# M-Igashi/mp3rgain

Measured on AMD Instinct MI355X. Metric: stereo PCM samples/s through IIR+RMS+histogram, higher is better.
Workload: dtype f64

## Files before the change

mp3rgain_amd/csrc/rg_k2_tm.hip:

```cpp
#include <hip/hip_runtime.h>

#include <atomic>
#include <type_traits>

#include "rg_device.h"
#include "rg_device_inl.h"

#include "rg_tm.h"

namespace {

__device__ __forceinline__ double tm_step(double (&s)[10], double (&t)[2], const double x, const RgTmCoef &K) {
    const double y = fma(K.b[0], x, s[0]);
#pragma unroll
    for (int i = 0; i < 9; ++i) s[i] = fma(-K.a[i + 1], y, fma(K.b[i + 1], x, s[i + 1]));
    s[9] = fma(-K.a[10], y, fma(K.b[10], x, K.c0));
    const double z = fma(K.bb[0], y, t[0]);
    t[0] = fma(-K.ba[1], z, fma(K.bb[1], y, t[1]));
    t[1] = fma(-K.ba[2], z, fma(K.bb[2], y, K.c0));
    return z;
}

__device__ __forceinline__ double tm_step_servo(double (&s)[10], double (&t)[2], const double x, const RgTmCoef &K) {
    const double y = fma(K.b[0], x, s[0]);
#pragma unroll
    for (int i = 0; i < 9; ++i) s[i] = fma(-K.a[i + 1], y, fma(K.b[i + 1], x, s[i + 1]));
    s[9] = fma(-K.a[10], y, K.b[10] * x);
    const double z = y - t[0];
    const double p = t[0] + t[1];
    t[1] = fma(K.beta, z, t[1]);
    t[0] = fma(K.alpha, z, p);
    return z;
}

template <int NCH>
struct TmLane {
    double s[NCH][10];
    double t[NCH][2];
    double A[NCH];
    double B[NCH][RG_TM_DIM];
};

typedef __attribute__((address_space(4))) const double rg_cdouble;

template <int NCH, int NX>
__device__ __forceinline__ void tm_sample(TmLane<NCH> &st, const double (&x)[NCH], rg_cdouble *__restrict__ Trow,
                                          const RgTmCoef &K) {
#pragma unroll
    for (int c = 0; c < NCH; ++c) {
        const double z = tm_step(st.s[c], st.t[c], x[c], K);
        st.A[c] = fma(z, z, st.A[c]);
#pragma unroll
        for (int j = RG_TM_DIM - NX; j < RG_TM_DIM; ++j) st.B[c][j] = fma(z, Trow[j], st.B[c][j]);
    }
}

template <int FMT> struct Fmt;
template <> struct Fmt<RG_FMT_F32_PLANAR> {
    typedef float elem;
    typedef float peak_t;
    static __device__ __forceinline__ double cvt(float v, float &pk) { pk = fmaxf(pk, fabsf(v)); return (double)v; }
    static __device__ __forceinline__ double peak_norm(float pk) { return (double)pk; }
    static __device__ __forceinline__ float peak_denorm(double v) { return (float)v; }
    static __device__ __forceinline__ uint32_t word(float v) { return __float_as_uint(v); }
    static __device__ __forceinline__ double cvt_word(uint32_t w, float &pk) { return cvt(__uint_as_float(w), pk); }
    static __device__ __forceinline__ void peak4(const uint32_t (&f)[4], float &pk) {
        pk = fmaxf(fmaxf(pk, fabsf(__uint_as_float(f[0]))), fabsf(__uint_as_float(f[1])));
        pk = fmaxf(fmaxf(pk, fabsf(__uint_as_float(f[2]))), fabsf(__uint_as_float(f[3])));
    }
    static __device__ __forceinline__ double word_value(uint32_t w) { return (double)__uint_as_float(w); }
};
template <> struct Fmt<RG_FMT_S16_PLANAR> {
    typedef int16_t elem;
    typedef uint32_t peak_t;
    static __device__ __forceinline__ double cvt(int16_t v, uint32_t &pk) {
        const int32_t w = v;
        const uint32_t m = (uint32_t)(w < 0 ? -w : w);
        pk = m > pk ? m : pk;
        return (double)w;
    }
    static __device__ __forceinline__ double peak_norm(uint32_t pk) { return (double)pk / 32768.0; }
    static __device__ __forceinline__ uint32_t peak_denorm(double v) { return (uint32_t)(v * 32768.0); }
    static __device__ __forceinline__ uint32_t word(int16_t v) { return (uint32_t)(int32_t)v; }
    static __device__ __forceinline__ double cvt_word(uint32_t w, uint32_t &pk) { return cvt((int16_t)(int32_t)w, pk); }
    static __device__ __forceinline__ void peak4(const uint32_t (&f)[4], uint32_t &pk) {
#pragma unroll
        for (int u = 0; u < 4; ++u) (void)cvt_word(f[u], pk);
    }
    static __device__ __forceinline__ double word_value(uint32_t w) { return (double)(int32_t)w; }
};
template <> struct Fmt<RG_FMT_S32_PLANAR> {
    typedef int32_t elem;
    typedef uint32_t peak_t;
    static __device__ __forceinline__ double cvt(int32_t v, uint32_t &pk) {
        const uint32_t m = v < 0 ? (uint32_t)0 - (uint32_t)v : (uint32_t)v;
        pk = m > pk ? m : pk;
        return (double)v;
    }
    static __device__ __forceinline__ double peak_norm(uint32_t pk) { return (double)pk / 2147483648.0; }
    static __device__ __forceinline__ uint32_t peak_denorm(double v) { return (uint32_t)(v * 2147483648.0); }
    static __device__ __forceinline__ uint32_t word(int32_t v) { return (uint32_t)v; }
    static __device__ __forceinline__ double cvt_word(uint32_t w, uint32_t &pk) { return cvt((int32_t)w, pk); }
    static __device__ __forceinline__ void peak4(const uint32_t (&f)[4], uint32_t &pk) {
#pragma unroll
        for (int u = 0; u < 4; ++u) (void)cvt_word(f[u], pk);
    }
    static __device__ __forceinline__ double word_value(uint32_t w) { return (double)(int32_t)w; }
};

template <typename T>
__device__ __forceinline__ uint32_t find_track(const RgTmTrack *__restrict__ tracks, uint32_t n_tracks, uint32_t block,
                                               T RgTmTrack::*base) {
    uint32_t lo = 0, hi = n_tracks - 1;
    while (lo < hi) {
        const uint32_t mid = (lo + hi + 1) >> 1;
        if (tracks[mid].*base <= block) lo = mid; else hi = mid - 1;
    }
    return lo;
}

}

#define RG_TM_TILE 16

typedef uint32_t __attribute__((ext_vector_type(4))) rg_u32x4;
typedef uint32_t __attribute__((ext_vector_type(4), aligned(4))) rg_u32x4u;
typedef short __attribute__((ext_vector_type(4), aligned(2))) rg_s16x4u;

template <int FMT, int NX, bool MASK, bool PEAK = true, bool SERVO = false>
__device__ __forceinline__ void tm_frame(TmLane<1> &st, const uint32_t wbits, typename Fmt<FMT>::peak_t &pk,
                                         const double *__restrict__ tr , const RgTmCoef &K,
                                         const uint32_t n, const uint32_t len) {
    double (&s)[10] = st.s[0];
    double (&t)[2] = st.t[0];
    const double x = PEAK ? Fmt<FMT>::cvt_word(wbits, pk) : Fmt<FMT>::word_value(wbits);
#ifdef RG_TM_LOADER_ONLY
    st.A[0] += x;
    return;
#endif
    if constexpr (SERVO) {
        const double y = fma(K.b[0], x, s[0]);
        double u[10];
#pragma unroll
        for (int i = 0; i < 9; ++i) u[i] = fma(K.b[i + 1], x, s[i + 1]);
        u[9] = K.b[10] * x;
        const double p = t[0] + t[1];
        __builtin_amdgcn_sched_barrier(0);
        double z = y - t[0];
#pragma unroll
        for (int i = 0; i < 10; ++i) s[i] = fma(-K.a[i + 1], y, u[i]);
        __builtin_amdgcn_sched_barrier(0);
        if (MASK) z = n < len ? z : 0.0;
        t[1] = fma(K.beta, z, t[1]);
        t[0] = fma(K.alpha, z, p);
        st.A[0] = fma(z, z, st.A[0]);
#pragma unroll
        for (int j = 0; j < NX; ++j) st.B[0][RG_TM_DIM - NX + j] = fma(z, tr[j], st.B[0][RG_TM_DIM - NX + j]);
        __builtin_amdgcn_sched_barrier(0);
        return;
    }
    const double y = fma(K.b[0], x, s[0]);
    double u[10];
#pragma unroll
    for (int i = 0; i < 9; ++i) u[i] = fma(K.b[i + 1], x, s[i + 1]);
    u[9] = fma(K.b[10], x, K.c0);
    __builtin_amdgcn_sched_barrier(0);
    double z = fma(K.bb[0], y, t[0]);
    const double w1 = fma(K.bb[1], y, t[1]);
    const double w2 = fma(K.bb[2], y, K.c0);
    __builtin_amdgcn_sched_barrier(0);
#pragma unroll
    for (int i = 0; i < 10; ++i) s[i] = fma(-K.a[i + 1], y, u[i]);
    __builtin_amdgcn_sched_barrier(0);
    t[0] = fma(-K.ba[1], z, w1);
    t[1] = fma(-K.ba[2], z, w2);
    if (MASK) z = n < len ? z : 0.0;
    st.A[0] = fma(z, z, st.A[0]);
#pragma unroll
    for (int j = 0; j < NX; ++j) st.B[0][RG_TM_DIM - NX + j] = fma(z, tr[j], st.B[0][RG_TM_DIM - NX + j]);
    __builtin_amdgcn_sched_barrier(0);
}

template <int NX>
__device__ __forceinline__ void tm_load_row(double (&dst)[NX], const double *__restrict__ src) {
#pragma unroll
    for (int j = 0; j < NX; j += 2) {
        const double2 v = *reinterpret_cast<const double2 *>(src + j);
        dst[j] = v.x;
        dst[j + 1] = v.y;
    }
}

template <int FMT, bool TAIL, bool MOM, bool SERVO>
__device__ __forceinline__ void tm_fast_path(TmLane<1> &st, typename Fmt<FMT>::peak_t &pk, const RgTmCoef &K, const uint32_t L,
                                             const uint32_t H,
                                             const __attribute__((address_space(1))) typename Fmt<FMT>::elem *rowp,
                                             const uint32_t len,
                                             const double *__restrict__ T12, const double *__restrict__ T2,
                                             char *const wtile ) {
    typedef Fmt<FMT> F;
    typedef const __attribute__((address_space(1))) typename F::elem gelem;
    const int lane = threadIdx.x & 63;
#ifdef RG_TM_LINEWIDE
    constexpr bool kLineWide = !MOM && !TAIL && FMT == RG_FMT_F32_PLANAR;
#else
    constexpr bool kLineWide = false;
#endif
    const int lrow = lane >> 2, lslot = lane & 3;
    gelem *lfirst[4];
    uint32_t llen[4];
#pragma unroll
    for (int q = 0; q < 4; ++q) {
        const int row = 16 * q + lrow;
        const int piece = lslot ^ ((row >> 2) & 3);
        const unsigned long long base = __shfl((unsigned long long)(uintptr_t)rowp, row, 64);
        lfirst[q] = (gelem *)(uintptr_t)base + 4u * piece;
        llen[q] = L;
        if (TAIL) llen[q] = __shfl(len, row, 64);
    }
    const char *const rrow = wtile + lane * 64;
    const char *const rrow1 = wtile + RG_TM_WAVE_TILE_BYTES + (kLineWide ? lane ^ 1 : lane) * 64;
    const int rswz = (lane >> 2) & 3;
    const uint32_t ntiles = (L + RG_TM_TILE - 1) / RG_TM_TILE;

    constexpr int NSTAGE = MOM ? 1 : 2;
    rg_u32x4 stage[NSTAGE][4];
    auto load4 = [&](gelem *src) -> rg_u32x4 {
        if constexpr (FMT == RG_FMT_S16_PLANAR) {
            const rg_s16x4u v = *(const __attribute__((address_space(1))) rg_s16x4u *)src;
            return rg_u32x4{(uint32_t)(int32_t)v.x, (uint32_t)(int32_t)v.y, (uint32_t)(int32_t)v.z, (uint32_t)(int32_t)v.w};
        } else {
            return *(const __attribute__((address_space(1))) rg_u32x4u *)src;
        }
    };
    auto load_tile = [&](uint32_t tile, auto buf, auto whole) {
        constexpr int SB = decltype(buf)::value;
        constexpr bool WHOLE = decltype(whole)::value;
        const uint32_t n0 = tile * RG_TM_TILE;
#pragma unroll
        for (int q = 0; q < 4; ++q) {
            const int row = 16 * q + lrow;
            const int piece = lslot ^ ((row >> 2) & 3);
            const uint32_t pn = n0 + 4u * piece;
            if (!TAIL) {
                if (WHOLE || n0 + RG_TM_TILE <= L || pn < L) stage[SB][q] = load4(lfirst[q] + n0);
            } else {
                gelem *src = lfirst[q] + n0;
                if (pn + 4u <= llen[q]) {
                    stage[SB][q] = load4(src);
                } else {
                    stage[SB][q].x = pn + 0u < llen[q] ? F::word(src[0]) : 0u;
                    stage[SB][q].y = pn + 1u < llen[q] ? F::word(src[1]) : 0u;
                    stage[SB][q].z = pn + 2u < llen[q] ? F::word(src[2]) : 0u;
                    stage[SB][q].w = pn + 3u < llen[q] ? F::word(src[3]) : 0u;
                }
            }
        }
    };
    auto store_tile = [&](auto buf) {
        constexpr int SB = decltype(buf)::value;
        __builtin_amdgcn_wave_barrier();
#pragma unroll
        for (int q = 0; q < 4; ++q)
            *reinterpret_cast<uint4 *>(wtile + SB * RG_TM_WAVE_TILE_BYTES + q * 1024 + (lane ^ (kLineWide && SB ? 4 : 0)) * 16) =
                make_uint4(stage[SB][q].x, stage[SB][q].y, stage[SB][q].z, stage[SB][q].w);
        __builtin_amdgcn_fence(__ATOMIC_RELEASE, "wavefront");
        __builtin_amdgcn_wave_barrier();
    };
    auto read_piece = [&](int p, int slot) -> uint4 { return *reinterpret_cast<const uint4 *>((slot ? rrow1 : rrow) + 16 * (p ^ rswz)); };

    auto compute_tile = [&](const uint32_t tile, auto mode, auto buf) {
        constexpr int MODE = decltype(mode)::value;
        constexpr int SLOT = decltype(buf)::value;
        const uint32_t n0 = tile * RG_TM_TILE;
        const int np = (MODE != 0 && MODE != 4) ? 4 : (L - n0 >= RG_TM_TILE ? 4 : (int)((L - n0) >> 2));
        auto piece = [&](const int p, const uint4 v) {
            const uint32_t f[4] = {v.x, v.y, v.z, v.w};
            const uint32_t n = n0 + 4u * p;
            F::peak4(f, pk);
            if (MODE == 3 || MODE == 4) {
#pragma unroll
                for (int u = 0; u < 4; ++u) tm_frame<FMT, 0, TAIL, false, SERVO>(st, f[u], pk, nullptr, K, n + u, len);
            } else if (MODE == 1 || (MODE == 0 && n < H)) {
#pragma unroll
                for (int u = 0; u < 4; ++u) {
                    double row[12];
                    tm_load_row<12>(row, T12 + (size_t)(n + u) * 12);
                    tm_frame<FMT, 12, TAIL, false, SERVO>(st, f[u], pk, row, K, n + u, len);
                }
            } else {
                double rows[8];
                tm_load_row<4>(reinterpret_cast<double (&)[4]>(rows[0]), T2 + (size_t)(n - H) * 2);
                tm_load_row<4>(reinterpret_cast<double (&)[4]>(rows[4]), T2 + (size_t)(n - H) * 2 + 4);
#pragma unroll
                for (int u = 0; u < 4; ++u) {
                    const double tr[2] = {rows[2 * u], rows[2 * u + 1]};
                    tm_frame<FMT, 2, TAIL, false, SERVO>(st, f[u], pk, tr, K, n + u, len);
                }
            }
        };
        if constexpr (MODE != 0 && MODE != 4) {
            uint4 v[4];
            v[0] = read_piece(0, SLOT);
#pragma unroll
            for (int p = 0; p < 4; ++p) {
                if (p + 1 < 4) v[p + 1] = read_piece(p + 1, SLOT);
                piece(p, v[p]);
            }
        } else {
            uint4 v = make_uint4(0u, 0u, 0u, 0u);
            if (np) v = read_piece(0, SLOT);
#pragma unroll 1
            for (int p = 0; p < np; ++p) {
                const uint4 vn = p + 1 < np ? read_piece(p + 1, SLOT) : v;
                piece(p, v);
                v = vn;
            }
        }
        if ((MODE == 0 || MODE == 4) && tile + 1 == ntiles) {
            for (uint32_t n = L & ~3u; n < L; ++n) {
                const uint32_t o = n - n0;
                const uint32_t f = *reinterpret_cast<const uint32_t *>((SLOT ? rrow1 : rrow) + 16 * ((int)(o >> 2) ^ rswz) + 4 * (o & 3));
                if (MODE == 4) {
                    tm_frame<FMT, 0, TAIL, true, SERVO>(st, f, pk, nullptr, K, n, len);
                } else if (n < H) {
                    double row[12];
                    tm_load_row<12>(row, T12 + (size_t)n * 12);
                    tm_frame<FMT, 12, TAIL, true, SERVO>(st, f, pk, row, K, n, len);
                } else {
                    const double tr[2] = {T2[(size_t)(n - H) * 2], T2[(size_t)(n - H) * 2 + 1]};
                    tm_frame<FMT, 2, TAIL, true, SERVO>(st, f, pk, tr, K, n, len);
                }
            }
        }
    };
    typedef std::integral_constant<int, 0> Mixed;
    typedef std::integral_constant<int, 1> All12;
    typedef std::integral_constant<int, 2> All2;
    typedef std::integral_constant<int, 3> None;
    typedef std::integral_constant<int, 4> NoneRagged;

    typedef std::integral_constant<int, 0> S0;
    typedef std::integral_constant<int, NSTAGE - 1> S1;
    typedef std::false_type Guarded;
    typedef std::true_type Whole;
    auto run_tile = [&](const uint32_t tile, auto mode, auto buf) {
        store_tile(buf);
        if (tile + NSTAGE < ntiles) load_tile(tile + NSTAGE, buf, Guarded{});
        compute_tile(tile, mode, buf);
    };
    const uint32_t full_tiles = L / RG_TM_TILE;
    uint32_t tile = 0;
    if constexpr (MOM) load_tile(0, S0{}, Guarded{});
    if constexpr (!MOM) {
        if constexpr (kLineWide) {
            const int wrow = lane >> 3, wslot = (lane >> 2) & 1, wpos = lane & 3;
            unsigned long long lo64 = (unsigned long long)(uintptr_t)rowp;
#pragma unroll
            for (int d = 32; d >= 1; d >>= 1) {
                const unsigned long long o = __shfl_xor(lo64, d, 64);
                lo64 = o < lo64 ? o : lo64;
            }
            const unsigned long long wbase = __builtin_amdgcn_readfirstlane((uint32_t)lo64) | ((unsigned long long)__builtin_amdgcn_readfirstlane((uint32_t)(lo64 >> 32)) << 32);
            const unsigned long long delta = (unsigned long long)(uintptr_t)rowp - wbase;
            const bool near = __all(delta < (1ull << 31)) && full_tiles >= 4;
            if (near) {
                uint32_t woff[8];
#pragma unroll
                for (int q = 0; q < 8; ++q) {
                    const int row = 8 * q + wrow;
                    woff[q] = __shfl((uint32_t)delta, row, 64) + 64u * wslot + 16u * (wpos ^ ((row >> 2) & 3));
                }
                const __attribute__((address_space(1))) char *const gb = (const __attribute__((address_space(1))) char *)(uintptr_t)wbase;
                auto pair_load = [&](const uint32_t t0) {
#pragma unroll
                    for (int q = 0; q < 8; ++q)
                        stage[q >> 2][q & 3] = *(const __attribute__((address_space(1))) rg_u32x4u *)(gb + (size_t)t0 * (RG_TM_TILE * 4) + woff[q]);
                };
                auto pair_store = [&]() {
                    __builtin_amdgcn_wave_barrier();
#pragma unroll
                    for (int q = 0; q < 8; ++q)
                        *reinterpret_cast<uint4 *>(wtile + wslot * RG_TM_WAVE_TILE_BYTES + ((8 * q + wrow) ^ wslot) * 64 + wpos * 16) =
                            make_uint4(stage[q >> 2][q & 3].x, stage[q >> 2][q & 3].y, stage[q >> 2][q & 3].z, stage[q >> 2][q & 3].w);
                    __builtin_amdgcn_fence(__ATOMIC_RELEASE, "wavefront");
                    __builtin_amdgcn_wave_barrier();
                };
                pair_load(0);
                for (; tile + 3 < full_tiles; tile += 2) {
                    pair_store();
                    if (tile + 5 < full_tiles) {
                        pair_load(tile + 2);
                    } else {
                        load_tile(tile + 2, S0{}, Guarded{});
                        if (tile + 3 < ntiles) load_tile(tile + 3, S1{}, Guarded{});
                    }
                    compute_tile(tile, None{}, S0{});
                    compute_tile(tile + 1, None{}, S1{});
                }
            } else {
                load_tile(0, S0{}, Guarded{});
                if (ntiles > 1) load_tile(1, S1{}, Guarded{});
                for (; tile + 3 < full_tiles; tile += 2) {
                    store_tile(S0{});
                    store_tile(S1{});
                    load_tile(tile + 2, S0{}, Whole{});
                    load_tile(tile + 3, S1{}, Whole{});
                    compute_tile(tile, None{}, S0{});
                    compute_tile(tile + 1, None{}, S1{});
                }
            }
        } else {
        load_tile(0, S0{}, Guarded{});
        if (ntiles > 1) load_tile(1, S1{}, Guarded{});
        for (; tile + 3 < full_tiles; tile += 2) {
            store_tile(S0{});
            store_tile(S1{});
            load_tile(tile + 2, S0{}, Whole{});
            load_tile(tile + 3, S1{}, Whole{});
            compute_tile(tile, None{}, S0{});
            compute_tile(tile + 1, None{}, S1{});
        }
        }
        while (tile < ntiles) {
            if (tile < full_tiles) run_tile(tile, None{}, S0{}); else run_tile(tile, NoneRagged{}, S0{});
            if (++tile >= ntiles) break;
            if (tile < full_tiles) run_tile(tile, None{}, S1{}); else run_tile(tile, NoneRagged{}, S1{});
            ++tile;
        }
        return;
    }
    const uint32_t t12 = (H / RG_TM_TILE) < full_tiles ? H / RG_TM_TILE : full_tiles;
    for (; tile < t12; ++tile) run_tile(tile, All12{}, S0{});
    if (tile < ntiles && (tile * RG_TM_TILE < H || tile >= full_tiles)) { run_tile(tile, Mixed{}, S0{}); ++tile; }
    for (; tile < full_tiles; ++tile) run_tile(tile, All2{}, S0{});
    for (; tile < ntiles; ++tile) run_tile(tile, Mixed{}, S0{});
}

template <int FMT, bool MULTI, bool SERVO>
__global__ void __launch_bounds__(MULTI ? RG_TM_BLOCK_WIDE_MULTI : RG_TM_BLOCK_WIDE)
rg_tm_main_kernel(const RgTmCoef K, const RgTmGeom G, const RgTmTrack *__restrict__ tracks, uint32_t n_tracks,
                  double *__restrict__ rec, uint32_t total_recs, double *__restrict__ win_energy ,
                  uint32_t total_windows, uint32_t *__restrict__ nonfinite, uint32_t lds_tables,
                  uint32_t *__restrict__ zero_words, uint64_t zero_count ,
                  unsigned long long *__restrict__ dbg ) {
    typedef Fmt<FMT> F;
    const unsigned long long dbg_t0 = dbg ? wall_clock64() : 0ull;
    const unsigned long long dbg_c0 = dbg ? __builtin_readcyclecounter() : 0ull;
    typedef typename F::elem elem;
    typedef __attribute__((address_space(1))) const elem gelem;
    extern __shared__ __attribute__((aligned(16))) char smem[];

    if (zero_words) {
        const uint64_t stride = (uint64_t)gridDim.x * blockDim.x;
        for (uint64_t w = (uint64_t)blockIdx.x * blockDim.x + threadIdx.x; w < zero_count; w += stride) zero_words[w] = 0u;
    }
    const uint32_t gl = blockIdx.x * blockDim.x + threadIdx.x;
    const uint32_t t = find_track(tracks, n_tracks, gl, &RgTmTrack::lane_base);
    struct { const void *ch0, *ch1; uint64_t frames; uint32_t nseg; } tr;
    {
        const RgTmTrack &q = tracks[t];
        tr.ch0 = q.ch0; tr.ch1 = q.ch1; tr.frames = q.frames; tr.nseg = q.nseg;
    }
    const uint32_t rel = gl - tracks[t].lane_base;
    const int chan = (tr.ch1 != nullptr && rel >= tr.nseg) ? 1 : 0;
    const uint32_t seg = rel - (chan ? tr.nseg : 0u);
    const uint32_t L = G.L;
    const uint32_t H = G.H10;
    const uint32_t m = MULTI ? G.m : 1u;
    const uint64_t seg_stride = (uint64_t)L * m;
    const bool active = seg < tr.nseg;
    const uint64_t start = (uint64_t)seg * seg_stride;
    uint32_t len = 0;
    if (active) {
        const uint64_t rem = tr.frames - start;
        len = rem < L ? (uint32_t)rem : L;
    }
    gelem *const chp = (gelem *)(chan == 0 ? tr.ch0 : tr.ch1);
    rg_cdouble *__restrict__ T = (rg_cdouble *)G.T;

    TmLane<1> st;
#pragma unroll
    for (int i = 0; i < 10; ++i) st.s[0][i] = 0.0;
    st.t[0][0] = st.t[0][1] = 0.0;
    st.A[0] = 0.0;
#pragma unroll
    for (int j = 0; j < RG_TM_DIM; ++j) st.B[0][j] = 0.0;
    typename F::peak_t pk = 0;
    auto rec_ptr = [&]() -> double * { return rec + (size_t)chan * RG_TM_REC * total_recs + ((size_t)tracks[t].rec_base + (active ? seg : 0)); };
    auto note_nonfinite = [&](const double energy, const uint32_t unit, const bool counts) {
        const bool bad = counts && !(fabs(energy) <= 1.7976931348623157e308);
        if (__any(bad) && bad) atomicMax(&nonfinite[tracks[t].track_index], 0xFFFFFFFFu - unit);
    };

    auto first_energy = [&]() -> double {
        if constexpr (SERVO) return fabs(st.A[0]) <= 1.7976931348623157e308 ? st.A[0] + fma(K.aff_lin, st.t[0][1], K.aff_n * (double)len) : st.A[0];
        return st.A[0];
    };
    bool done = false;
    {
        if (lds_tables) {
            done = true;
            const uint32_t tbl_doubles = H * 12 + (L - H) * 2;
            {
                const double2 *__restrict__ src = reinterpret_cast<const double2 *>(G.Tlds);
                double2 *dst = reinterpret_cast<double2 *>(smem);
                const uint32_t n16 = tbl_doubles / 2;
                const uint32_t BS = blockDim.x;
                uint32_t i = threadIdx.x;
                for (; i + 3 * BS < n16; i += 4 * BS) {
                    const double2 a = src[i], b = src[i + BS], c = src[i + 2 * BS], d = src[i + 3 * BS];
                    dst[i] = a;
                    dst[i + BS] = b;
                    dst[i + 2 * BS] = c;
                    dst[i + 3 * BS] = d;
                }
                for (; i < n16; i += BS) dst[i] = src[i];
                __syncthreads();
            }
            const double *const T12 = reinterpret_cast<const double *>(smem);
            const double *const T2 = T12 + (size_t)H * 12;
            char *const wtile = smem + (size_t)tbl_doubles * sizeof(double) + (threadIdx.x >> 6) * (RG_TM_WAVE_TILE_BYTES * (MULTI ? 2 : 1));
            const bool plain = len == L && start + ((L + 3u) & ~3u) <= tr.frames;
            if (__all(plain))
                tm_fast_path<FMT, false, true, SERVO>(st, pk, K, L, H, chp + start, len, T12, T2, wtile);
            else if (__any(len != 0))
                tm_fast_path<FMT, true, true, SERVO>(st, pk, K, L, H, chp + start, len, T12, T2, wtile);
            if constexpr (MULTI) {
                note_nonfinite(st.A[0], seg * m, active);
                if (active) {
                    double *__restrict__ const r = rec_ptr();
                    r[0] = first_energy();
#pragma unroll
                    for (int j = 0; j < RG_TM_DIM; ++j) r[(size_t)(1 + j) * total_recs] = st.B[0][j];
                }
#pragma unroll 1
                for (uint32_t w = 1; w < m; ++w) {
                    const uint64_t wstart = start + (uint64_t)w * L;
                    uint32_t lenw = 0;
                    if (active && wstart < tr.frames) {
                        const uint64_t rem = tr.frames - wstart;
                        lenw = rem < L ? (uint32_t)rem : L;
                    }
                    if (!__any(lenw != 0)) break;
                    st.A[0] = 0.0;
                    const double v2_start = st.t[0][1];
                    const bool idle = lenw == 0 && tr.frames >= (uint64_t)((L + 3u) & ~3u);
                    const bool plainw = idle || (lenw == L && wstart + ((L + 3u) & ~3u) <= tr.frames);
                    gelem *const rowp = idle ? chp : chp + wstart;
                    if (__all(plainw))
                        tm_fast_path<FMT, false, false, SERVO>(st, pk, K, L, H, rowp, lenw, T12, T2, wtile);
                    else
                        tm_fast_path<FMT, true, false, SERVO>(st, pk, K, L, H, rowp, lenw, T12, T2, wtile);
                    note_nonfinite(st.A[0], seg * m + w, lenw != 0);
                    double energy = st.A[0];
                    if constexpr (SERVO) energy = fabs(energy) <= 1.7976931348623157e308 ? energy + fma(K.aff_lin, st.t[0][1] - v2_start, K.aff_n * (double)lenw) : energy;
                    if (lenw != 0) win_energy[(size_t)chan * total_windows + tracks[t].win_base + (size_t)seg * m + w] = energy;
                }
            }
        }
    }
    if (!done) {
        gelem *const p0 = chp + start;
        for (uint32_t n = 0; n < L; ++n) {
            const bool valid = n < len;
            double x = 0.0;
            if (valid) x = F::cvt(p0[n], pk);
            rg_cdouble *__restrict__ Trow = T + (size_t)n * RG_TM_DIM;
            double z;
            if constexpr (SERVO) {
                const double v2 = st.t[0][1];
                z = tm_step_servo(st.s[0], st.t[0], x, K);
                if (!valid) st.t[0][1] = v2;
            } else {
                z = tm_step(st.s[0], st.t[0], x, K);
            }
            z = valid ? z : 0.0;
            st.A[0] = fma(z, z, st.A[0]);
#pragma unroll
            for (int j = 0; j < RG_TM_DIM; ++j) st.B[0][j] = fma(z, Trow[j], st.B[0][j]);
        }
    }

    if (dbg && (threadIdx.x & 63) == 0) {
        const size_t w = ((size_t)blockIdx.x * (blockDim.x / 64) + (threadIdx.x >> 6)) * 6;
        dbg[w + 4] = dbg_c0;
        dbg[w + 5] = __builtin_readcyclecounter();
        dbg[w + 0] = dbg_t0;
        dbg[w + 1] = wall_clock64();
        dbg[w + 2] = ((unsigned long long)__builtin_amdgcn_s_getreg((20 << 0) | (0 << 6) | (31 << 11)) << 32) |
                     __builtin_amdgcn_s_getreg((4 << 0) | (0 << 6) | (31 << 11));
        dbg[w + 3] = done ? 1ull : 0ull;
    }

    if constexpr (!MULTI) {
        note_nonfinite(st.A[0], seg, active);
        if (active) {
            double *__restrict__ const r = rec_ptr();
            r[0] = first_energy();
#pragma unroll
            for (int j = 0; j < RG_TM_DIM; ++j) r[(size_t)(1 + j) * total_recs] = st.B[0][j];
        }
    }
    if (active) {
        double *__restrict__ const r = rec_ptr();
#pragma unroll
        for (int j = 0; j < 10; ++j) r[(size_t)(13 + j) * total_recs] = st.s[0][j];
        r[(size_t)23 * total_recs] = st.t[0][0];
        r[(size_t)24 * total_recs] = st.t[0][1];
        r[(size_t)25 * total_recs] = F::peak_norm(pk);
    }
}


template <typename V>
__device__ __forceinline__ void tm_performed(V old) {
    asm volatile("" ::"v"(old));
}

template <typename GP>
__device__ __forceinline__ double tm_quad_half(GP Gm, const double (&sg)[RG_TM_DIM]) {
    double quad = 0.0;
    int p = 0;
#pragma unroll
    for (int j = 0; j < RG_TM_DIM; ++j) {
        double row = 0.5 * Gm[p] * sg[j];
        ++p;
#pragma unroll
        for (int q = j + 1; q < RG_TM_DIM; ++q, ++p) row = fma(Gm[p], sg[q], row);
        quad = fma(row, sg[j], quad);
    }
    return quad;
}

template <int NCH>
__global__ void __launch_bounds__(RG_TM_BLOCK)
rg_tm_fix_kernel(const RgTmGeom G, const RgTmFixTables FT, const RgTmTrack *__restrict__ tracks, uint32_t n_tracks,
                 const double *__restrict__ rec, uint32_t total_recs,
                 const double *__restrict__ win_energy , uint32_t total_windows,
                 uint32_t *__restrict__ nonfinite,
                 uint32_t *__restrict__ imprecise, uint32_t *__restrict__ hist,
                 unsigned long long *__restrict__ peak_bits, uint32_t *__restrict__ done_count,
                 rg_track_result *__restrict__ results,
                 unsigned long long *__restrict__ dbg ) {
#define TM_FIX_STAMP(k)                                                            \
    do {                                                                           \
        if (dbg && threadIdx.x == 0) dbg[(size_t)blockIdx.x * 8 + (k)] = wall_clock64(); \
    } while (0)
    __builtin_amdgcn_s_setprio(3);
    TM_FIX_STAMP(0);
    __shared__ double edge[RG_TM_BLOCK / 64][RG_TM_EDGE][NCH * RG_TM_DIM];
    __shared__ uint64_t pct_scan[RG_PCT_THREADS];
    __shared__ double pieces[RG_TM_BLOCK];
    __shared__ double pieces_m[RG_TM_BLOCK];
    __shared__ double pieces_e[RG_TM_BLOCK];
    __shared__ int is_last;
    __shared__ double part_sg[NCH][RG_TM_DIM];
    __shared__ uint32_t part_len;
    __shared__ int part_lane;
    const int lane = threadIdx.x & 63, wave = threadIdx.x >> 6;
    if (threadIdx.x == 0) part_len = 0;
    auto publish_edge = [&](const double x, const int slot) {
        if (lane >= 64 - RG_TM_EDGE) edge[wave][lane - (64 - RG_TM_EDGE)][slot] = x;
    };
    auto from_below = [&](const double x, const int d, const int slot) -> double {
        double v = __shfl_up(x, d, 64);
        if (lane < d) v = wave > 0 ? edge[wave - 1][RG_TM_EDGE - d + lane][slot] : 0.0;
        return v;
    };

    const uint32_t t = find_track(tracks, n_tracks, blockIdx.x, &RgTmTrack::fix_block_base);
    const RgTmTrack tr = tracks[t];
    const uint32_t b = blockIdx.x - tr.fix_block_base;
    const int i = threadIdx.x;
    const int warm = (int)G.warm;
    const uint32_t NB = G.fix_windows * G.k;
    const long long seg = (long long)b * NB - warm + i;
    const bool in_block = i < warm + (int)NB;
    const bool seg_valid = in_block && seg >= 0 && seg < (long long)tr.nseg;
    const bool owner = seg_valid && i >= warm;
    const size_t idx = (size_t)tr.rec_base + (size_t)(seg_valid ? seg : 0);
    __shared__ double ftab[RG_TM_GRAM + RG_TM_MAX_ROUNDS * 104 + 36 + 100 + 12];
    {
        const double *__restrict__ src = FT.Gp + (size_t)(G.L - 1) * RG_TM_GRAM;
        const int n = RG_TM_GRAM + (int)G.rounds * 104 + 36 + (G.servo ? 112 : (G.whiten ? 100 : 0));
        for (int q = i; q < n; q += RG_TM_BLOCK) ftab[q] = src[q];
    }
    const double *const Gfull = ftab;
    const double *const PhiY = ftab + RG_TM_GRAM;
    const double *const PhiB = PhiY + G.rounds * 100;
    const double *const X = PhiB + G.rounds * 4;
    const double *const S0 = X + 24;
    const double *const Wf = S0 + 12;
    const double *const STf = Wf + 100;

    double w[NCH][RG_TM_DIM], pk = 0.0;
#pragma unroll
    for (int c = 0; c < NCH; ++c) {
        const double *__restrict__ r = rec + (size_t)c * RG_TM_REC * total_recs + idx;
#pragma unroll
        for (int j = 0; j < RG_TM_DIM; ++j) w[c][j] = seg_valid ? r[(size_t)(13 + j) * total_recs] : 0.0;
    }
    __syncthreads();
    TM_FIX_STAMP(1);
    const bool vstart = in_block && seg == -1;
#pragma unroll
    for (int c = 0; c < NCH; ++c) {
        double tq[2];
#pragma unroll
        for (int q = 0; q < 2; ++q) {
            double acc = G.whiten ? fma(X[q * 12 + 10], w[c][10], X[q * 12 + 11] * w[c][11]) : w[c][10 + q];
#pragma unroll
            for (int j = 0; j < 10; ++j) acc = fma(X[q * 12 + j], w[c][j], acc);
            tq[q] = acc;
        }
        w[c][10] = tq[0];
        w[c][11] = tq[1];
        if (G.whiten) {
#pragma unroll
            for (int i = 0; i < 10; ++i) {
                double acc = 0.0;
#pragma unroll
                for (int j = 0; j < 10; ++j)
                    if (j >= i) acc = fma(Wf[i * 10 + j], w[c][j], acc);
                w[c][i] = acc;
            }
        }
        if (vstart) {
#pragma unroll
            for (int j = 0; j < RG_TM_DIM; ++j) w[c][j] = S0[j];
        }
    }
    for (uint32_t rd = 0; rd < G.rounds; ++rd) {
        const int d = 1 << rd;
        const bool fast = rd < G.rounds_fast;
        double wn[NCH][RG_TM_DIM];
#pragma unroll
        for (int c = 0; c < NCH; ++c)
#pragma unroll
            for (int j = 0; j < RG_TM_DIM; ++j)
                if (j >= 10 || fast) publish_edge(w[c][j], c * RG_TM_DIM + j);
        __syncthreads();
#pragma unroll
        for (int c = 0; c < NCH; ++c)
#pragma unroll
            for (int j = 0; j < RG_TM_DIM; ++j) wn[c][j] = (j >= 10 || fast) ? from_below(w[c][j], d, c * RG_TM_DIM + j) : 0.0;
        __syncthreads();
        if (fast) {
            const double *PY = PhiY + (size_t)rd * 100;
#pragma unroll
            for (int a = 0; a < 10; ++a) {
                double py[10];
#pragma unroll
                for (int q = 0; q < 10; ++q) py[q] = PY[a * 10 + q];
#pragma unroll
                for (int c = 0; c < NCH; ++c) {
                    double acc = w[c][a];
#pragma unroll
                    for (int q = 0; q < 10; ++q) acc = fma(py[q], wn[c][q], acc);
                    w[c][a] = acc;
                }
                if (a & 1) __builtin_amdgcn_sched_barrier(0);
            }
        }
        const double *PB = PhiB + (size_t)rd * 4;
#pragma unroll
        for (int c = 0; c < NCH; ++c) {
            w[c][10] = fma(PB[0], wn[c][10], fma(PB[1], wn[c][11], w[c][10]));
            w[c][11] = fma(PB[2], wn[c][10], fma(PB[3], wn[c][11], w[c][11]));
        }
    }
#pragma unroll
    for (int c = 0; c < NCH; ++c)
#pragma unroll
        for (int j = 0; j < RG_TM_DIM; ++j) publish_edge(w[c][j], c * RG_TM_DIM + j);
    __syncthreads();
    double sgm[NCH][RG_TM_DIM];
#pragma unroll
    for (int c = 0; c < NCH; ++c)
#pragma unroll
        for (int j = 0; j < RG_TM_DIM; ++j) sgm[c][j] = from_below(w[c][j], 1, c * RG_TM_DIM + j);

    TM_FIX_STAMP(2);
    double S = 0.0, Mseg = 0.0, Eseg = 0.0;
    if (owner) {
        const uint64_t start = (uint64_t)seg * G.L * G.m;
        const uint64_t rem = tr.frames - start;
        const uint32_t len = rem < G.L ? (uint32_t)rem : G.L;
        const bool full = len == G.L;
        double lin[NCH], quad[NCH];
#pragma unroll
        for (int c = 0; c < NCH; ++c) {
            const double *__restrict__ r = rec + (size_t)c * RG_TM_REC * total_recs + idx;
            double acc = 0.0;
#pragma unroll
            for (int j = 0; j < RG_TM_DIM; ++j) acc = fma(r[(size_t)(1 + j) * total_recs], sgm[c][j], acc);
            lin[c] = acc;
            quad[c] = 0.0;
            pk = fmax(pk, r[(size_t)25 * total_recs]);
            S += r[0];
            Mseg += r[0];
            double st = 0.0;
#pragma unroll
            for (int j = 0; j < 10; ++j) st = fma(fabs(sgm[c][j]), G.tau10[j], st);
            Eseg = fma(2.0 * st, sqrt(fabs(r[0])) * 1.0001, Eseg);
        }
        if (full) {
#pragma unroll
            for (int j = 0; j < RG_TM_DIM; ++j) {
                const int p = j * RG_TM_DIM - (j * (j - 1)) / 2 - j;
                double g[RG_TM_DIM];
#pragma unroll
                for (int q = 0; q < RG_TM_DIM; ++q)
                    if (q >= j) g[q] = Gfull[p + q];
#pragma unroll
                for (int c = 0; c < NCH; ++c) {
                    double row = 0.5 * g[j] * sgm[c][j];
#pragma unroll
                    for (int q = 0; q < RG_TM_DIM; ++q)
                        if (q > j) row = fma(g[q], sgm[c][q], row);
                    quad[c] = fma(row, sgm[c][j], quad[c]);
                }
                __builtin_amdgcn_sched_barrier(0);
            }
        } else {
#pragma unroll
            for (int c = 0; c < NCH; ++c)
#pragma unroll
                for (int j = 0; j < RG_TM_DIM; ++j) part_sg[c][j] = sgm[c][j];
            part_len = len;
            part_lane = i;
        }
#pragma unroll
        for (int c = 0; c < NCH; ++c) {
            S += 2.0 * (lin[c] + quad[c]);
            Mseg += 2.0 * quad[c];
        }
        if (G.servo && full) {
            double aff = 0.0;
#pragma unroll
            for (int c = 0; c < NCH; ++c) {
                double sx = 0.0;
#pragma unroll
                for (int j = 0; j < RG_TM_DIM; ++j) sx = fma(STf[j], sgm[c][j], sx);
                aff = fma(G.aff_sig, sx, aff);
            }
            S += aff;
        }
    }
    const uint32_t nf = nonfinite[tr.track_index];
    if (nf != 0 && owner) {
        const uint64_t unit = (uint64_t)seg * G.m, bad = 0xFFFFFFFFu - nf;
        if (unit > bad) S = __longlong_as_double(0x7FF8000000000000ll);
        else if (unit == bad) {
            double cls = 0.0;
#pragma unroll
            for (int c = 0; c < NCH; ++c) {
                const double a = rec[(size_t)c * RG_TM_REC * total_recs + idx];
                if (!(fabs(a) <= 1.7976931348623157e308)) cls += a;
            }
// ... 214 lines not shown
```

Before: 452.5 billion.

## Stream follow-on windows continuously through one double-buffered tile pipeline

Replaces the per-window loop, which re-entered the tile pipeline for each window with its own prologue, drain and ragged tail, with a single streaming path that processes all subsequent windows of a segment as one continuous sample stream. Window boundaries and track ends are handled inside event tiles, and lanes whose tracks end are re-pinned to an idle pointer, so the steady loop keeps double-buffered whole-tile loads going across window edges. The fast path is simplified to the first-window momentum mode and the optional line-wide variant is removed. The cost is more complex boundary logic, with wave-wide votes and per-sample handling at window edges.

```diff
diff --git a/mp3rgain_amd/csrc/rg_k2_tm.hip b/mp3rgain_amd/csrc/rg_k2_tm.hip
--- a/mp3rgain_amd/csrc/rg_k2_tm.hip
+++ b/mp3rgain_amd/csrc/rg_k2_tm.hip
@@ -191,7 +191,7 @@
     }
 }
 
-template <int FMT, bool TAIL, bool MOM, bool SERVO>
+template <int FMT, bool TAIL, bool SERVO>
 __device__ __forceinline__ void tm_fast_path(TmLane<1> &st, typename Fmt<FMT>::peak_t &pk, const RgTmCoef &K, const uint32_t L,
                                              const uint32_t H,
                                              const __attribute__((address_space(1))) typename Fmt<FMT>::elem *rowp,
@@ -201,11 +201,6 @@
     typedef Fmt<FMT> F;
     typedef const __attribute__((address_space(1))) typename F::elem gelem;
     const int lane = threadIdx.x & 63;
-#ifdef RG_TM_LINEWIDE
-    constexpr bool kLineWide = !MOM && !TAIL && FMT == RG_FMT_F32_PLANAR;
-#else
-    constexpr bool kLineWide = false;
-#endif
     const int lrow = lane >> 2, lslot = lane & 3;
     gelem *lfirst[4];
     uint32_t llen[4];
@@ -219,11 +214,10 @@
         if (TAIL) llen[q] = __shfl(len, row, 64);
     }
     const char *const rrow = wtile + lane * 64;
-    const char *const rrow1 = wtile + RG_TM_WAVE_TILE_BYTES + (kLineWide ? lane ^ 1 : lane) * 64;
     const int rswz = (lane >> 2) & 3;
     const uint32_t ntiles = (L + RG_TM_TILE - 1) / RG_TM_TILE;
 
-    constexpr int NSTAGE = MOM ? 1 : 2;
+    constexpr int NSTAGE = 1;
     rg_u32x4 stage[NSTAGE][4];
     auto load4 = [&](gelem *src) -> rg_u32x4 {
         if constexpr (FMT == RG_FMT_S16_PLANAR) {
@@ -262,26 +256,23 @@
         __builtin_amdgcn_wave_barrier();
 #pragma unroll
         for (int q = 0; q < 4; ++q)
-            *reinterpret_cast<uint4 *>(wtile + SB * RG_TM_WAVE_TILE_BYTES + q * 1024 + (lane ^ (kLineWide && SB ? 4 : 0)) * 16) =
+            *reinterpret_cast<uint4 *>(wtile + SB * RG_TM_WAVE_TILE_BYTES + q * 1024 + lane * 16) =
                 make_uint4(stage[SB][q].x, stage[SB][q].y, stage[SB][q].z, stage[SB][q].w);
         __builtin_amdgcn_fence(__ATOMIC_RELEASE, "wavefront");
         __builtin_amdgcn_wave_barrier();
     };
-    auto read_piece = [&](int p, int slot) -> uint4 { return *reinterpret_cast<const uint4 *>((slot ? rrow1 : rrow) + 16 * (p ^ rswz)); };
+    auto read_piece = [&](int p, int) -> uint4 { return *reinterpret_cast<const uint4 *>(rrow + 16 * (p ^ rswz)); };
 
     auto compute_tile = [&](const uint32_t tile, auto mode, auto buf) {
         constexpr int MODE = decltype(mode)::value;
         constexpr int SLOT = decltype(buf)::value;
         const uint32_t n0 = tile * RG_TM_TILE;
-        const int np = (MODE != 0 && MODE != 4) ? 4 : (L - n0 >= RG_TM_TILE ? 4 : (int)((L - n0) >> 2));
+        const int np = MODE != 0 ? 4 : (L - n0 >= RG_TM_TILE ? 4 : (int)((L - n0) >> 2));
         auto piece = [&](const int p, const uint4 v) {
             const uint32_t f[4] = {v.x, v.y, v.z, v.w};
             const uint32_t n = n0 + 4u * p;
             F::peak4(f, pk);
-            if (MODE == 3 || MODE == 4) {
-#pragma unroll
-                for (int u = 0; u < 4; ++u) tm_frame<FMT, 0, TAIL, false, SERVO>(st, f[u], pk, nullptr, K, n + u, len);
-            } else if (MODE == 1 || (MODE == 0 && n < H)) {
+            if (MODE == 1 || (MODE == 0 && n < H)) {
 #pragma unroll
                 for (int u = 0; u < 4; ++u) {
                     double row[12];
@@ -299,7 +290,7 @@
                 }
             }
         };
-        if constexpr (MODE != 0 && MODE != 4) {
+        if constexpr (MODE != 0) {
             uint4 v[4];
             v[0] = read_piece(0, SLOT);
 #pragma unroll
@@ -317,13 +308,11 @@
                 v = vn;
             }
         }
-        if ((MODE == 0 || MODE == 4) && tile + 1 == ntiles) {
+        if (MODE == 0 && tile + 1 == ntiles) {
             for (uint32_t n = L & ~3u; n < L; ++n) {
                 const uint32_t o = n - n0;
-                const uint32_t f = *reinterpret_cast<const uint32_t *>((SLOT ? rrow1 : rrow) + 16 * ((int)(o >> 2) ^ rswz) + 4 * (o & 3));
-                if (MODE == 4) {
-                    tm_frame<FMT, 0, TAIL, true, SERVO>(st, f, pk, nullptr, K, n, len);
-                } else if (n < H) {
+                const uint32_t f = *reinterpret_cast<const uint32_t *>(rrow + 16 * ((int)(o >> 2) ^ rswz) + 4 * (o & 3));
+                if (n < H) {
                     double row[12];
                     tm_load_row<12>(row, T12 + (size_t)n * 12);
                     tm_frame<FMT, 12, TAIL, true, SERVO>(st, f, pk, row, K, n, len);
@@ -337,13 +326,9 @@
     typedef std::integral_constant<int, 0> Mixed;
     typedef std::integral_constant<int, 1> All12;
     typedef std::integral_constant<int, 2> All2;
-    typedef std::integral_constant<int, 3> None;
-    typedef std::integral_constant<int, 4> NoneRagged;
 
     typedef std::integral_constant<int, 0> S0;
-    typedef std::integral_constant<int, NSTAGE - 1> S1;
     typedef std::false_type Guarded;
-    typedef std::true_type Whole;
     auto run_tile = [&](const uint32_t tile, auto mode, auto buf) {
         store_tile(buf);
         if (tile + NSTAGE < ntiles) load_tile(tile + NSTAGE, buf, Guarded{});
@@ -351,90 +336,219 @@
     };
     const uint32_t full_tiles = L / RG_TM_TILE;
     uint32_t tile = 0;
-    if constexpr (MOM) load_tile(0, S0{}, Guarded{});
-    if constexpr (!MOM) {
-        if constexpr (kLineWide) {
-            const int wrow = lane >> 3, wslot = (lane >> 2) & 1, wpos = lane & 3;
-            unsigned long long lo64 = (unsigned long long)(uintptr_t)rowp;
-#pragma unroll
-            for (int d = 32; d >= 1; d >>= 1) {
-                const unsigned long long o = __shfl_xor(lo64, d, 64);
-                lo64 = o < lo64 ? o : lo64;
-            }
-            const unsigned long long wbase = __builtin_amdgcn_readfirstlane((uint32_t)lo64) | ((unsigned long long)__builtin_amdgcn_readfirstlane((uint32_t)(lo64 >> 32)) << 32);
-            const unsigned long long delta = (unsigned long long)(uintptr_t)rowp - wbase;
-            const bool near = __all(delta < (1ull << 31)) && full_tiles >= 4;
-            if (near) {
-                uint32_t woff[8];
-#pragma unroll
-                for (int q = 0; q < 8; ++q) {
-                    const int row = 8 * q + wrow;
-                    woff[q] = __shfl((uint32_t)delta, row, 64) + 64u * wslot + 16u * (wpos ^ ((row >> 2) & 3));
-                }
-                const __attribute__((address_space(1))) char *const gb = (const __attribute__((address_space(1))) char *)(uintptr_t)wbase;
-                auto pair_load = [&](const uint32_t t0) {
-#pragma unroll
-                    for (int q = 0; q < 8; ++q)
-                        stage[q >> 2][q & 3] = *(const __attribute__((address_space(1))) rg_u32x4u *)(gb + (size_t)t0 * (RG_TM_TILE * 4) + woff[q]);
-                };
-                auto pair_store = [&]() {
-                    __builtin_amdgcn_wave_barrier();
-#pragma unroll
-                    for (int q = 0; q < 8; ++q)
-                        *reinterpret_cast<uint4 *>(wtile + wslot * RG_TM_WAVE_TILE_BYTES + ((8 * q + wrow) ^ wslot) * 64 + wpos * 16) =
-                            make_uint4(stage[q >> 2][q & 3].x, stage[q >> 2][q & 3].y, stage[q >> 2][q & 3].z, stage[q >> 2][q & 3].w);
-                    __builtin_amdgcn_fence(__ATOMIC_RELEASE, "wavefront");
-                    __builtin_amdgcn_wave_barrier();
-                };
-                pair_load(0);
-                for (; tile + 3 < full_tiles; tile += 2) {
-                    pair_store();
-                    if (tile + 5 < full_tiles) {
-                        pair_load(tile + 2);
-                    } else {
-                        load_tile(tile + 2, S0{}, Guarded{});
-                        if (tile + 3 < ntiles) load_tile(tile + 3, S1{}, Guarded{});
-                    }
-                    compute_tile(tile, None{}, S0{});
-                    compute_tile(tile + 1, None{}, S1{});
-                }
-            } else {
-                load_tile(0, S0{}, Guarded{});
-                if (ntiles > 1) load_tile(1, S1{}, Guarded{});
-                for (; tile + 3 < full_tiles; tile += 2) {
-                    store_tile(S0{});
-                    store_tile(S1{});
-                    load_tile(tile + 2, S0{}, Whole{});
-                    load_tile(tile + 3, S1{}, Whole{});
-                    compute_tile(tile, None{}, S0{});
-                    compute_tile(tile + 1, None{}, S1{});
-                }
-            }
-        } else {
-        load_tile(0, S0{}, Guarded{});
-        if (ntiles > 1) load_tile(1, S1{}, Guarded{});
-        for (; tile + 3 < full_tiles; tile += 2) {
-            store_tile(S0{});
-            store_tile(S1{});
-            load_tile(tile + 2, S0{}, Whole{});
-            load_tile(tile + 3, S1{}, Whole{});
-            compute_tile(tile, None{}, S0{});
-            compute_tile(tile + 1, None{}, S1{});
-        }
-        }
-        while (tile < ntiles) {
-            if (tile < full_tiles) run_tile(tile, None{}, S0{}); else run_tile(tile, NoneRagged{}, S0{});
-            if (++tile >= ntiles) break;
-            if (tile < full_tiles) run_tile(tile, None{}, S1{}); else run_tile(tile, NoneRagged{}, S1{});
-            ++tile;
-        }
-        return;
-    }
+    load_tile(0, S0{}, Guarded{});
     const uint32_t t12 = (H / RG_TM_TILE) < full_tiles ? H / RG_TM_TILE : full_tiles;
     for (; tile < t12; ++tile) run_tile(tile, All12{}, S0{});
     if (tile < ntiles && (tile * RG_TM_TILE < H || tile >= full_tiles)) { run_tile(tile, Mixed{}, S0{}); ++tile; }
     for (; tile < full_tiles; ++tile) run_tile(tile, All2{}, S0{});
     for (; tile < ntiles; ++tile) run_tile(tile, Mixed{}, S0{});
+}
+
+template <int FMT, bool SERVO, typename GetPin, typename WindowDone>
+__device__ __forceinline__ void tm_stream_path(TmLane<1> &st, typename Fmt<FMT>::peak_t &pk, const RgTmCoef &K, const uint32_t L,
+                                               const uint32_t m,
+                                               const __attribute__((address_space(1))) typename Fmt<FMT>::elem *const sp ,
+                                               const uint32_t slen ,
+                                               GetPin &&get_pin ,
+                                               char *const wtile ,
+                                               WindowDone &&window_done ) {
+    typedef Fmt<FMT> F;
+    typedef const __attribute__((address_space(1))) typename F::elem gelem;
+    typedef const __attribute__((address_space(1))) char gbyte;
+    constexpr uint32_t EB = sizeof(typename F::elem);
+    constexpr uint32_t IDLE = 0xFFFFFFFFu;
+    const int lane = threadIdx.x & 63;
+    const uint32_t S = L * (m - 1);
+    auto is_live = [](const uint32_t v) { return v != 0u && v != IDLE; };
+    uint32_t vend = slen;
+    if (slen == 0) vend = get_pin() != nullptr ? IDLE : 0u;
+    bool any_dead = __any(vend == 0u);
+    const int lrow = lane >> 2, lslot = lane & 3;
+    gbyte *lptr[4];
+    uint32_t lstep[4];
+    uint32_t lt = 0;
+    {
+        gelem *const first = slen ? sp : get_pin();
+#pragma unroll
+        for (int q = 0; q < 4; ++q) {
+            const int row = 16 * q + lrow;
+            const int piece = lslot ^ ((row >> 2) & 3);
+            const unsigned long long base = __shfl((unsigned long long)(uintptr_t)first, row, 64);
+            lptr[q] = (gbyte *)(uintptr_t)base + 4u * EB * piece;
+            lstep[q] = __shfl(slen, row, 64) ? 2u * RG_TM_TILE * EB : 0u;
+        }
+    }
+    const char *const rrow = wtile + lane * 64;
+    const int rswz = (lane >> 2) & 3;
+
+    rg_u32x4 stage[2][4];
+    auto load4 = [&](gelem *src) -> rg_u32x4 {
+        if constexpr (FMT == RG_FMT_S16_PLANAR) {
+            const rg_s16x4u v = *(const __attribute__((address_space(1))) rg_s16x4u *)src;
+            return rg_u32x4{(uint32_t)(int32_t)v.x, (uint32_t)(int32_t)v.y, (uint32_t)(int32_t)v.z, (uint32_t)(int32_t)v.w};
+        } else {
+            return *(const __attribute__((address_space(1))) rg_u32x4u *)src;
+        }
+    };
+    auto load_tile = [&](auto dt, auto buf, auto whole) {
+        constexpr int DT = decltype(dt)::value;
+        constexpr int SB = decltype(buf)::value;
+        constexpr bool WHOLE = decltype(whole)::value;
+        const uint32_t n0 = (lt + DT) * RG_TM_TILE;
+        if (!WHOLE && n0 >= S) return;
+#pragma unroll
+        for (int q = 0; q < 4; ++q) {
+            gelem *const src = (gelem *)(lptr[q] + DT * RG_TM_TILE * EB);
+            if (WHOLE) {
+                stage[SB][q] = load4(src);
+            } else {
+                const int row = 16 * q + lrow;
+                const int piece = lslot ^ ((row >> 2) & 3);
+                const uint32_t pn = n0 + 4u * piece;
+                const uint32_t llen = __shfl(vend, row, 64);
+                if (pn + 4u <= llen) {
+                    stage[SB][q] = load4(src);
+                } else {
+                    stage[SB][q].x = pn + 0u < llen ? F::word(src[0]) : 0u;
+                    stage[SB][q].y = pn + 1u < llen ? F::word(src[1]) : 0u;
+                    stage[SB][q].z = pn + 2u < llen ? F::word(src[2]) : 0u;
+                    stage[SB][q].w = pn + 3u < llen ? F::word(src[3]) : 0u;
+                }
+            }
+        }
+    };
+    auto advance = [&]() {
+#pragma unroll
+        for (int q = 0; q < 4; ++q) lptr[q] += lstep[q];
+        lt += 2;
+    };
+    auto store_tile = [&](auto buf) {
+        constexpr int SB = decltype(buf)::value;
+        __builtin_amdgcn_wave_barrier();
+#pragma unroll
+        for (int q = 0; q < 4; ++q)
+            *reinterpret_cast<uint4 *>(wtile + SB * RG_TM_WAVE_TILE_BYTES + q * 1024 + lane * 16) =
+                make_uint4(stage[SB][q].x, stage[SB][q].y, stage[SB][q].z, stage[SB][q].w);
+        __builtin_amdgcn_fence(__ATOMIC_RELEASE, "wavefront");
+        __builtin_amdgcn_wave_barrier();
+    };
+    auto compute_tile = [&](auto buf) {
+        constexpr int SLOT = decltype(buf)::value;
+        const char *const r = rrow + SLOT * RG_TM_WAVE_TILE_BYTES;
+        uint4 v[4];
+        v[0] = *reinterpret_cast<const uint4 *>(r + 16 * (0 ^ rswz));
+#pragma unroll
+        for (int p = 0; p < 4; ++p) {
+            if (p + 1 < 4) v[p + 1] = *reinterpret_cast<const uint4 *>(r + 16 * ((p + 1) ^ rswz));
+            const uint32_t f[4] = {v[p].x, v[p].y, v[p].z, v[p].w};
+            F::peak4(f, pk);
+#pragma unroll
+            for (int u = 0; u < 4; ++u) tm_frame<FMT, 0, false, false, SERVO>(st, f[u], pk, nullptr, K, 0u, 0u);
+        }
+    };
+
+    uint32_t w = 1;
+    uint32_t wbase = 0;
+    uint32_t bnext = L;
+    st.A[0] = 0.0;
+    double v2_start = st.t[0][1];
+
+    auto event_tile = [&](const uint32_t tile, const int slot) -> bool {
+        const uint32_t n0 = tile * RG_TM_TILE;
+        const char *const r = rrow + slot * RG_TM_WAVE_TILE_BYTES;
+        uint32_t o = 0;
+#pragma unroll 1
+        while (o < RG_TM_TILE) {
+            const uint32_t n = n0 + o;
+            if (n >= S) return true;
+            if ((o & 3u) == 0u && bnext >= n + 4u && __all(vend >= n + 4u)) {
+                const uint4 v = *reinterpret_cast<const uint4 *>(r + 16 * ((int)(o >> 2) ^ rswz));
+                const uint32_t f[4] = {v.x, v.y, v.z, v.w};
+                F::peak4(f, pk);
+#pragma unroll
+                for (int u = 0; u < 4; ++u) tm_frame<FMT, 0, false, false, SERVO>(st, f[u], pk, nullptr, K, 0u, 0u);
+                o += 4u;
+            } else {
+                const uint32_t f = *reinterpret_cast<const uint32_t *>(r + 16 * ((int)(o >> 2) ^ rswz) + 4 * (o & 3u));
+                tm_frame<FMT, 0, true, true, SERVO>(st, f, pk, nullptr, K, n, vend);
+                o += 1u;
+            }
+            if (n0 + o == bnext) {
+                const uint32_t rem = vend - wbase;
+                window_done(w, rem < L ? rem : L, is_live(vend) && vend > wbase, v2_start);
+                st.A[0] = 0.0;
+                v2_start = st.t[0][1];
+                wbase = bnext;
+                bnext += L;
+                if (++w == m) return true;
+            }
+        }
+        const bool ends = is_live(vend) && vend <= n0 + RG_TM_TILE;
+        if (__any(ends)) {
+            window_done(w, vend - wbase, ends && vend > wbase, v2_start);
+            gelem *const pin = get_pin();
+#pragma unroll
+            for (int q = 0; q < 4; ++q) {
+                const int row = 16 * q + lrow;
+                const int piece = lslot ^ ((row >> 2) & 3);
+                const unsigned long long base = __shfl((unsigned long long)(uintptr_t)pin, row, 64);
+                if (__shfl((int)ends, row, 64)) {
+                    lptr[q] = (gbyte *)(uintptr_t)base + 4u * EB * piece;
+                    lstep[q] = 0u;
+                }
+            }
+            if (ends) vend = pin != nullptr ? IDLE : 0u;
+            any_dead = __any(vend == 0u);
+        }
+        return false;
+    };
+    auto steady_limit = [&]() -> uint32_t {
+        if (any_dead) return 0u;
+        uint32_t f = is_live(vend) ? vend / RG_TM_TILE : IDLE;
+#pragma unroll
+        for (int d = 32; d >= 1; d >>= 1) {
+            const uint32_t o = __shfl_xor(f, d, 64);
+            f = o < f ? o : f;
+        }
+        f = __builtin_amdgcn_readfirstlane(f);
+        const uint32_t s = S / RG_TM_TILE, b = (bnext - 1u) / RG_TM_TILE + 2u;
+        f = f < s ? f : s;
+        return f < b ? f : b;
+    };
+
+    typedef std::integral_constant<int, 0> S0;
+    typedef std::integral_constant<int, 1> S1;
+    typedef std::integral_constant<int, 0> T0;
+    typedef std::integral_constant<int, 1> T1;
+    typedef std::false_type Guarded;
+    typedef std::true_type Whole;
+    load_tile(T0{}, S0{}, Guarded{});
+    load_tile(T1{}, S1{}, Guarded{});
+    advance();
+    uint32_t tile = 0;
+    uint32_t limit = steady_limit();
+    for (;;) {
+        for (; tile + 4u <= limit; tile += 2) {
+            store_tile(S0{});
+            store_tile(S1{});
+            load_tile(T0{}, S0{}, Whole{});
+            load_tile(T1{}, S1{}, Whole{});
+            advance();
+            compute_tile(S0{});
+            compute_tile(S1{});
+        }
+        store_tile(S0{});
+        store_tile(S1{});
+        load_tile(T0{}, S0{}, Guarded{});
+        load_tile(T1{}, S1{}, Guarded{});
+        advance();
+        bool last = false;
+#pragma unroll 1
+        for (int s = 0; s < 2 && !last; ++s) last = event_tile(tile + s, s);
+        tile += 2;
+        if (last || !__any(is_live(vend))) break;
+        limit = steady_limit();
+    }
 }
 
 template <int FMT, bool MULTI, bool SERVO>
@@ -523,9 +637,9 @@
             char *const wtile = smem + (size_t)tbl_doubles * sizeof(double) + (threadIdx.x >> 6) * (RG_TM_WAVE_TILE_BYTES * (MULTI ? 2 : 1));
             const bool plain = len == L && start + ((L + 3u) & ~3u) <= tr.frames;
             if (__all(plain))
-                tm_fast_path<FMT, false, true, SERVO>(st, pk, K, L, H, chp + start, len, T12, T2, wtile);
+                tm_fast_path<FMT, false, SERVO>(st, pk, K, L, H, chp + start, len, T12, T2, wtile);
             else if (__any(len != 0))
-                tm_fast_path<FMT, true, true, SERVO>(st, pk, K, L, H, chp + start, len, T12, T2, wtile);
+                tm_fast_path<FMT, true, SERVO>(st, pk, K, L, H, chp + start, len, T12, T2, wtile);
             if constexpr (MULTI) {
                 note_nonfinite(st.A[0], seg * m, active);
                 if (active) {
@@ -534,28 +648,24 @@
 #pragma unroll
                     for (int j = 0; j < RG_TM_DIM; ++j) r[(size_t)(1 + j) * total_recs] = st.B[0][j];
                 }
-#pragma unroll 1
-                for (uint32_t w = 1; w < m; ++w) {
-                    const uint64_t wstart = start + (uint64_t)w * L;
-                    uint32_t lenw = 0;
-                    if (active && wstart < tr.frames) {
-                        const uint64_t rem = tr.frames - wstart;
-                        lenw = rem < L ? (uint32_t)rem : L;
-                    }
-                    if (!__any(lenw != 0)) break;
-                    st.A[0] = 0.0;
-                    const double v2_start = st.t[0][1];
-                    const bool idle = lenw == 0 && tr.frames >= (uint64_t)((L + 3u) & ~3u);
-                    const bool plainw = idle || (lenw == L && wstart + ((L + 3u) & ~3u) <= tr.frames);
-                    gelem *const rowp = idle ? chp : chp + wstart;
-                    if (__all(plainw))
-                        tm_fast_path<FMT, false, false, SERVO>(st, pk, K, L, H, rowp, lenw, T12, T2, wtile);
-                    else
-                        tm_fast_path<FMT, true, false, SERVO>(st, pk, K, L, H, rowp, lenw, T12, T2, wtile);
-                    note_nonfinite(st.A[0], seg * m + w, lenw != 0);
-                    double energy = st.A[0];
-                    if constexpr (SERVO) energy = fabs(energy) <= 1.7976931348623157e308 ? energy + fma(K.aff_lin, st.t[0][1] - v2_start, K.aff_n * (double)lenw) : energy;
-                    if (lenw != 0) win_energy[(size_t)chan * total_windows + tracks[t].win_base + (size_t)seg * m + w] = energy;
+                const uint32_t S = L * (m - 1u);
+                uint32_t slen = 0;
+                if (active && start + L < tr.frames) {
+                    const uint64_t rem = tr.frames - (start + L);
+                    slen = rem < S ? (uint32_t)rem : S;
+                }
+                if (m > 1u && __any(slen != 0)) {
+                    auto get_pin = [&]() -> gelem * {
+                        const RgTmTrack &q = tracks[t];
+                        return q.frames >= 2u * RG_TM_TILE ? (gelem *)(chan == 0 ? q.ch0 : q.ch1) : nullptr;
+                    };
+                    auto window_done = [&](const uint32_t w, const uint32_t lenw, const bool stores, const double v2_start) {
+                        note_nonfinite(st.A[0], seg * m + w, stores);
+                        double energy = st.A[0];
+                        if constexpr (SERVO) energy = fabs(energy) <= 1.7976931348623157e308 ? energy + fma(K.aff_lin, st.t[0][1] - v2_start, K.aff_n * (double)lenw) : energy;
+                        if (stores) win_energy[(size_t)chan * total_windows + tracks[t].win_base + (size_t)seg * m + w] = energy;
+                    };
+                    tm_stream_path<FMT, SERVO>(st, pk, K, L, m, chp + start + L, slen, get_pin, wtile, window_done);
                 }
             }
         }
```

Result: no change. 456.3 billion, median of 6 (+0.8%).
